# WangXinyan940/openmm-chargeflux

Measured on AMD Instinct MI355X. Metric: ns/day + ms/force-eval, periodic charge-flux box, 1/2/4/8 MI355X, higher is better.
Workload: dtype f64; 1 GPU; C3: periodic flexible charge-flux water box, 96000 atoms, Ewald rc=1.0 nm tol=0.0001 (alpha 2.91842, kmax 31, K_half 113490), velocity Verlet dt=1 fs, fp64; atoms=96000, k_half=113490, handover=event, variants=0, kspace=grid (ES kernel W=13, pruned DFT), same k-set, parallelism=atom-decomposition x1

## Files before the change

### openmm-chargeflux_amd/csrc/cf_api.hip

```cpp
#include <hip/hip_runtime.h>

#include <algorithm>
#include <cmath>
#include <cstring>
#include <exception>
#include <numeric>
#include <stdexcept>
#include <string>
#include <vector>

#include "cf_internal.h"

enum Phase { PH_FLUX, PH_PREP, PH_CELLS, PH_NLIST, PH_TABLES, PH_SFAC, PH_COEFFS, PH_FORCE, PH_DIRECT,
             PH_ASSEMBLE, PH_ENERGY, PH_GSORT, PH_GSPREAD, PH_GDFTF, PH_GDFTI, PH_GINTERP, PH_EXCL, PH_COUNT };
static const char* kPhaseNames[PH_COUNT] = {"flux_terms", "atoms_prep", "cell_sort", "neighbor_list",
                                            "kspace_tables", "kspace_sfac", "kspace_coeffs", "kspace_force",
                                            "direct_pairs", "assemble", "energy", "grid_sort", "grid_spread",
                                            "grid_dft_fwd", "grid_dft_inv", "grid_interp", "direct_excl"};
constexpr int kMaxTimed = 8192;

static void graph_forget(cf_handle* H);
static void graph_invalidate(cf_handle* H);
struct GraphCache;
static GraphCache* graph_active(cf_handle* H);
// ... 147 lines not shown

void set_cells(cf_handle* H, const double L[3]) {
    cf::Handle& h = H->h;
    const double bx = h.box_t[0], cx = h.box_t[1], cy = h.box_t[2];
    const double V = L[0] * L[1] * L[2];
    const double width[3] = {V / std::sqrt((L[1] * L[2]) * (L[1] * L[2]) + (bx * L[2]) * (bx * L[2]) +
                                           (bx * cy - L[1] * cx) * (bx * cy - L[1] * cx)),
                             L[1] * L[2] / std::sqrt(L[2] * L[2] + cy * cy), L[2]};
    int nc[3];
    for (int d = 0; d < 3; d++) {
        double v = std::floor((h.tric ? width[d] : L[d]) / (h.cutoff + h.list_skin));
        nc[d] = (int)std::max(1.0, std::min(v, 1024.0));
    }
    int64_t ncell = (int64_t)nc[0] * nc[1] * nc[2];
    if (ncell > h.ncell_alloc) {
        bump_epoch(H);
        if (h.cell_start) { free_idle(h, h.cell_start); free_idle(h, h.cell_end); free_idle(h, h.cell_cnt); }
        if (h.own_cnt) { free_idle(h, h.own_cnt); free_idle(h, h.own_start); h.own_cnt = h.own_start = nullptr; }
        zalloc((void**)&h.cell_start, sizeof(int) * ncell, "cells");
        zalloc((void**)&h.cell_end, sizeof(int) * ncell, "cells");
        zalloc((void**)&h.cell_cnt, sizeof(int) * ncell, "cells");
        if (h.world > 1) {
            zalloc((void**)&h.own_cnt, sizeof(int) * ncell, "cells");
            zalloc((void**)&h.own_start, sizeof(int) * (ncell + 1), "cells");
        }
        h.ncell_alloc = (int)ncell;
    }
    h.nc[0] = nc[0]; h.nc[1] = nc[1]; h.nc[2] = nc[2];
    if (h.nl) alloc_nlist(H, h.list_skin, L[0] * L[1] * L[2]);
    const double per_cell = (double)h.n / (double)ncell;
    const bool want_cluster = h.pair_list == CF_PAIR_LIST_CLUSTER || h.pair_list == CF_PAIR_LIST_AUTO;
    h.half = h.pair_list != CF_PAIR_LIST_FULL && h.pbc &&
             (h.world == 1 || (want_cluster && h.pair_list == CF_PAIR_LIST_CLUSTER)) && nc[0] >= 4 &&
             nc[1] >= 4 && nc[2] >= 4 && per_cell * 18.0 * 1.15 <= 4096.0 && h.n < (1 << 21);
    if (h.half && ncell > h.win_cells) {
        if (h.win_out) { free_idle(h, h.win_out); free_idle(h, h.win_woff); }
        zalloc((void**)&h.win_out, sizeof(unsigned long long) * 4 * 4096 * (size_t)ncell, "half-list windows");
        zalloc((void**)&h.win_woff, sizeof(int) * 18 * (size_t)ncell, "half-list windows");
        h.win_cells = (int)ncell;
        bump_epoch(H);
    }
    h.cluster = h.half && want_cluster;
    h.zcol = 0;
    if (h.cluster) {
        h.zcol = (int)std::max(1.0, std::min(8.0, std::round(std::sqrt(per_cell / 12.0))));
        const int need = h.n / 4 + (int)ncell + 1;
        const double rho = h.n / V;
        const double ext = 0.6 * std::cbrt(4.0 / rho);
        const double rl = h.cutoff + h.list_skin + ext;
        const double est = 0.5 * 4.0 / 3.0 * M_PI * rl * rl * rl * rho / 4.0 + 8.0;
        int cap = std::min(1536, ((int)(2.2 * est) + 64 + 15) / 16 * 16);
        if (h.list_capacity > 0) cap = std::max(4, std::min(cap, h.list_capacity));
        if (need > h.ncl_cap || cap != h.cpl_cap || ncell + 1 > h.cl_cells) {
            if (h.cl_start) { free_idle(h, h.cl_start); free_idle(h, h.cl_info); free_idle(h, h.cl_bb);
                              free_idle(h, h.cpl); free_idle(h, h.cpl_cnt); }
            h.ncl_cap = std::max(need, h.ncl_cap);
            h.cpl_cap = cap;
            h.cl_cells = std::max((int)ncell + 1, h.cl_cells);
            zalloc((void**)&h.cl_start, sizeof(int) * h.cl_cells, "cluster table");
            zalloc((void**)&h.cl_info, sizeof(int2) * h.ncl_cap, "cluster table");
            zalloc((void**)&h.cl_bb, sizeof(float4) * 2 * h.ncl_cap, "cluster table");
            zalloc((void**)&h.cpl, sizeof(uint2) * ((size_t)h.ncl_cap * h.cpl_cap + 64), "cluster-pair list");
            zalloc((void**)&h.cpl_cnt, sizeof(int) * h.ncl_cap, "cluster-pair list");
            bump_epoch(H);
        }
        if (!h.pos4f) {
            zalloc((void**)&h.pos4f, sizeof(float4) * (h.n + 4), "fp32 positions");
            zalloc((void**)&h.slot_of, sizeof(int) * h.n, "slot map");
            bump_epoch(H);
        }
    }
}

void set_box(cf_handle* H, const double* box9) {
    cf::Handle& h = H->h;
    if (!h.pbc) { h.box_L[0] = h.box_L[1] = h.box_L[2] = 1.0; return; }
    if (!box9) fail(CF_ERR_INVALID, "periodic box required");
    check_box_reduced(box9, "current box");
    double L[3] = {box9[0], box9[4], box9[8]};
    for (int d = 0; d < 3; d++)
        if (h.cutoff > 0.5 * L[d] * (1 + 1e-12))
            fail(CF_ERR_INVALID, "cutoff exceeds half the periodic box (minimum image would be ambiguous)");
    h.box_L[0] = L[0]; h.box_L[1] = L[1]; h.box_L[2] = L[2];
    h.box_t[0] = box9[3]; h.box_t[1] = box9[6]; h.box_t[2] = box9[7];
    h.tric = box9[3] != 0 || box9[6] != 0 || box9[7] != 0;
}

void partition(const cf_params* p, int world, int rank, int* lo, int* hi) {
    const int n = p->num_particles;
    if (world <= 1) { *lo = 0; *hi = n; return; }
    std::vector<int> par(n);
    std::iota(par.begin(), par.end(), 0);
    auto unite = [&](int a, int b) {
        if (a < 0 || a >= n || b < 0 || b >= n) fail(CF_ERR_INVALID, "particle index out of range");
        a = find_root(par, a); b = find_root(par, b);
        if (a != b) par[std::max(a, b)] = std::min(a, b);
    };
    for (int t = 0; t < p->num_flux_bonds; t++) unite(p->flux_bond_idx[2 * t], p->flux_bond_idx[2 * t + 1]);
    for (int t = 0; t < p->num_flux_angles; t++) {
        unite(p->flux_angle_idx[3 * t], p->flux_angle_idx[3 * t + 1]);
        unite(p->flux_angle_idx[3 * t], p->flux_angle_idx[3 * t + 2]);
    }
    for (int t = 0; t < p->num_flux_waters; t++) {
        unite(p->flux_water_idx[3 * t], p->flux_water_idx[3 * t + 1]);
        unite(p->flux_water_idx[3 * t], p->flux_water_idx[3 * t + 2]);
    }
    for (int k = 0; k < p->num_exceptions; k++) unite(p->exceptions[2 * k], p->exceptions[2 * k + 1]);
    std::vector<int> cmax(n, 0);
    for (int i = 0; i < n; i++) { int r = find_root(par, i); cmax[r] = std::max(cmax[r], i); }
    std::vector<char> valid(n + 1, 0);
    valid[0] = valid[n] = 1;
    int pm = -1;
    for (int c = 1; c < n; c++) {
        pm = std::max(pm, cmax[find_root(par, c - 1)]);
// ... 364 lines not shown
                h.g_t2 = dalloc<double2>(H, (size_t)gp.ng[0] * gp.NY * gp.KZ);
                h.g_b = dalloc<double2>(H, (size_t)gp.NX * gp.NY * gp.KZ);
                h.g_cnt = dalloc<int>(H, gp.nbins);
                check_hip(hipMemset(h.g_cnt, 0, sizeof(int) * gp.nbins), "memset");
                h.g_start = dalloc<int>(H, gp.nbins + 1);
                const size_t no = std::max(nown, 1);
                h.g_srec = dalloc<double4>(H, no);
                h.g_g0u = dalloc<int4>(H, no);
                h.g_rank = dalloc<int>(H, no);
                h.g_tmp = dalloc<int>(H, no);
                h.g_order = dalloc<int>(H, no);
                h.g_g0s = dalloc<int4>(H, no);
                h.g_taps = dalloc<double>(H, no * 72);
                check_hip(hipMemset(h.g_taps, 0, sizeof(double) * no * 72), "memset taps");
                if (h.world > 1) {
                    h.g_xrange = dalloc<int>(H, 3 + 2 * ((size_t)no / 256 + 1));
                    const int init[3] = {INT_MAX, INT_MIN, 0};
                    check_hip(hipMemcpy(h.g_xrange, init, sizeof(init), hipMemcpyHostToDevice), "x-slab init");
                }
                h.t_part = dalloc<double>(H, no * 4);
                h.e_rec_part = dalloc<double>(H, std::max<size_t>((size_t)(gp.NX * gp.NY * gp.KZ + 255) / 256,
                                                                  (size_t)gp.NY * gp.KZ / 16 + 2) + 1);
            } else {
                int blocks_k = (int)((h.khalf + 255) / 256);
                h.sk_nchunk = std::max(1, std::min((2048 + blocks_k - 1) / blocks_k, std::max(1, nown / 256)));
                h.kvec = dalloc<double4>(H, h.khalf);
                h.sk_slab = dalloc<double>(H, (size_t)h.sk_nchunk * 2 * h.khalf);
                h.sk_red = dalloc<double>(H, (size_t)2 * h.khalf);
                h.t_part = dalloc<double>(H, (size_t)nown * 4);
                h.e_rec_part = dalloc<double>(H, (size_t)(h.khalf + 255) / 256 + 1);
            }
        }
        check_hip(hipDeviceSynchronize(), "create sync");
        *out = H;
    });
    if (rc != CF_OK && H) {
        for (void* p2 : H->allocs) (void)hipFree(p2);
        if (H->h.err_host) (void)hipHostFree(H->h.err_host);
        delete H;
    }
    return rc;
}

CF_EXPORT int cf_destroy(cf_handle* H) {
    if (!H) return CF_OK;
    return guarded([&] {
        (void)hipSetDevice(H->h.device);
        drain_handle(H->h);
        graph_forget(H);
        for (void* p : H->allocs) (void)hipFree(p);
        for (auto& v : H->ev)
            for (hipEvent_t e : v) (void)hipEventDestroy(e);
        if (H->h.win_out) { (void)hipFree(H->h.win_out); (void)hipFree(H->h.win_woff); }
        if (H->h.cl_start) { (void)hipFree(H->h.cl_start); (void)hipFree(H->h.cl_info); (void)hipFree(H->h.cl_bb);
                             (void)hipFree(H->h.cpl); (void)hipFree(H->h.cpl_cnt); }
        if (H->h.pos4f) { (void)hipFree(H->h.pos4f); (void)hipFree(H->h.slot_of); }
        if (H->h.cell_start) (void)hipFree(H->h.cell_start);
        if (H->h.cell_end) (void)hipFree(H->h.cell_end);
        if (H->h.cell_cnt) (void)hipFree(H->h.cell_cnt);
        if (H->h.own_cnt) { (void)hipFree(H->h.own_cnt); (void)hipFree(H->h.own_start); }
        if (H->h.own_stream) (void)hipStreamDestroy(H->h.stream);
        if (H->h.aux) (void)hipStreamDestroy(H->h.aux);
        if (H->h.ev_fork) (void)hipEventDestroy(H->h.ev_fork);
        if (H->h.ev_join) (void)hipEventDestroy(H->h.ev_join);
        if (H->h.err_host) (void)hipHostFree(H->h.err_host);
        delete H;
    });
}

CF_EXPORT int cf_partition(const cf_params* p, int32_t world_size, int32_t rank, int32_t* lo, int32_t* hi) {
    return guarded([&] {
        if (!p || !lo || !hi) fail(CF_ERR_INVALID, "null argument");
        if (p->num_particles <= 0) fail(CF_ERR_INVALID, "num_particles must be > 0");
        int world = world_size <= 1 ? 1 : world_size;
        if (rank < 0 || rank >= world) fail(CF_ERR_INVALID, "rank out of range");
        int l = 0, h = 0;
        partition(p, world, rank, &l, &h);
        *lo = l; *hi = h;
    });
}

CF_EXPORT int cf_set_neighbor_skin(cf_handle* H, double skin) {
    return guarded([&] {
        if (!H) fail(CF_ERR_INVALID, "null handle");
        if (!(skin >= 0 && skin < 1e3)) fail(CF_ERR_INVALID, "skin must be finite and >= 0");
        cf::Handle& h = H->h;
        if (h.pending_flags >= 0) fail(CF_ERR_STATE, "cf_set_neighbor_skin during a begun evaluation");
        check_hip(hipSetDevice(h.device), "hipSetDevice");
        check_hip(hipStreamSynchronize(h.stream), "stream sync");
        h.skin = skin;
        h.list_valid = false;
        bump_epoch(H);
        if (!h.pbc) return;
        alloc_nlist(H, skin);
        if (skin > 0 && !h.pos_ref) h.pos_ref = dalloc<double>(H, (size_t)3 * h.n);
    });
}

CF_EXPORT int cf_update_parameters(cf_handle* H, const cf_params* p) {
    return guarded([&] {
        if (!H || !p) fail(CF_ERR_INVALID, "null argument");
        cf::Handle& h = H->h;
        if (h.pending_flags >= 0) fail(CF_ERR_STATE, "cf_update_parameters during a begun evaluation");
        if (p->num_particles != h.n) fail(CF_ERR_INVALID, "the number of particles has changed");
        if ((p->use_pbc ? 1 : 0) != h.pbc) fail(CF_ERR_INVALID, "periodicity cannot be changed by an update");
        if (h.pbc && (p->cutoff != h.cutoff || p->ewald_tol != h.tol))
            fail(CF_ERR_INVALID, "the cutoff and Ewald tolerance cannot be changed by an update");
// ... 865 lines not shown
```

### openmm-chargeflux_amd/csrc/cf_internal.h

```cpp
#pragma once

#include <hip/hip_runtime.h>
#include <stdint.h>

#include <string>
#include <vector>

#include "../../include/chargeflux.h"

namespace cf {

constexpr double kPi = 3.14159265358979323846;

struct KGeom {
    int KX = 0, KY = 0, KZ = 0;
    int NY = 0;
    int NYB = 0;
    int NYP = 0;
    int NYB4 = 0;
    int NMT = 0;
    int NZP = 0;
    int NB = 0;
    int CSW = 0;
    __host__ __device__ int nslots() const { return KX * NYP; }
// ... 88 lines not shown
    hipEvent_t ev_fork = nullptr, ev_join = nullptr;
    unsigned long long* sync_flag = nullptr;
    unsigned long long sync_seq = 0, join_seq = 0;
    bool handover_memory = false;
    double* dedq_rec = nullptr;
    double* f_rec = nullptr;
    int ncell_alloc = 0;
    int nc[3] = {0, 0, 0};
    int* cell_key = nullptr; int* cell_key_sorted = nullptr;
    int* atom_val = nullptr; int* atom_sorted = nullptr;
    int* cell_start = nullptr; int* cell_end = nullptr; int* cell_cnt = nullptr;
    double4* pos4s = nullptr;
    double2* ljs = nullptr;
    int lj_ntypes = 0;
    int* atom_type = nullptr;
    int* typ_s = nullptr;
    double2* lj_tab = nullptr;
    double skin = 0.0;
    double list_skin = 0.0;
    double list_L[3] = {0, 0, 0};
    double list_T[3] = {0, 0, 0};
    bool list_valid = false;
    double* pos_ref = nullptr;
    int* skin_flag = nullptr;
    long long* n_builds_dev = nullptr;
    long long* n_fallback_dev = nullptr;
    int64_t n_evals = 0;
    int* err_dev = nullptr;
    int* err_host = nullptr;
    int* err_host_dev = nullptr;
    int* key_tmp = nullptr; int* atom_tmp = nullptr;
    int* own_s = nullptr;
    int* own_cnt = nullptr;
    int* own_start = nullptr;
    int nb_cap = 0;
    int* nl = nullptr;
    int* nl_cnt = nullptr;
    bool half = false;
    int64_t alloc_epoch = 0;
    int* half_flag = nullptr;
    unsigned long long* win_out = nullptr;
    int* win_woff = nullptr;
    int win_cells = 0;
    bool cluster = false;
    int pair_list = CF_PAIR_LIST_AUTO;
    int list_capacity = 0;
    int variants = 0;
    int block_rounds() const { return (variants >> 8) & 15; }
    int zcol = 0;
    int ncl_cap = 0;
    int cl_cells = 0;
    int* cl_start = nullptr;
    int2* cl_info = nullptr;
    float4* cl_bb = nullptr;
    int cpl_cap = 0;
    uint2* cpl = nullptr;
    int* cpl_cnt = nullptr;
    float4* pos4f = nullptr;
    int* slot_of = nullptr;
    int npad = 0;
    double2* tab_xq = nullptr;
    double2* tab_y = nullptr;
    double* tab_cs = nullptr;
    double* s_slab = nullptr;
    double* s_red = nullptr;
    double* coef_a = nullptr;
    double* t_part = nullptr;
    double* e_rec_part = nullptr;
    int e_rec_nblk = 0;
    int coef_inv = 0;
    GridPlan gp;
    double* g_grid = nullptr;
    double2* g_t1 = nullptr;
    double2* g_t2 = nullptr;
    double2* g_b = nullptr;
    double2* g_tw[3] = {nullptr, nullptr, nullptr};
    double2* g_tw8[3] = {nullptr, nullptr, nullptr};
    double* g_deconv[3] = {nullptr, nullptr, nullptr};
    int* g_cnt = nullptr;
    int* g_start = nullptr;
    double4* g_srec = nullptr;
    int4* g_g0u = nullptr;
    int* g_rank = nullptr;
    int* g_tmp = nullptr;
    int* g_order = nullptr;
    int4* g_g0s = nullptr;
    double* g_taps = nullptr;
    int* g_xrange = nullptr;
    int64_t khalf = 0;
    double* sk_slab = nullptr;
    double* sk_red = nullptr;
    double4* kvec = nullptr;
    int sk_nchunk = 0;
    double* erfc_tab = nullptr;
    double erfc_scale = 0; int erfc_m = 0;
    double erfc_scale_f = 0; int erfc_m_f = 0;
    float* erfc_tab_f = nullptr;
    double* terms_dev = nullptr;
    double* e_part = nullptr;
    double* energy_dev = nullptr;
    int* e_ticket = nullptr;
    int pending_flags = -1;
    bool direct_done = false;
    double box_L[3] = {0, 0, 0};
    double box_t[3] = {0, 0, 0};
    bool tric = false;
};

std::vector<double> erfc_table(double xmax, double* scale, int* m);
std::vector<float> erfc_table_f(double xmax, double* scale, int* m);
std::vector<double> erfc_table_deg(double xmax, int deg, double width, int max_m, double* scale, int* m);
void launch_flux_terms(Handle& h, const double* pos);
void launch_atoms_prep(Handle& h, const double* pos, bool skin_check);
void launch_cell_sort(Handle& h, const double* pos);
void launch_force_rebuild(Handle& h);
void launch_zero(Handle& h, double* p, int64_t n);
void launch_nlist(Handle& h, const double* pos);
void launch_cluster_list(Handle& h);
void launch_pairs_cluster(Handle& h, const double* pos, int include_forces);
void launch_cluster_table(Handle& h);
void launch_direct(Handle& h, const double* pos, int include_forces);
void launch_direct_finish(Handle& h, const double* pos, int include_forces);
void launch_recip_add(Handle& h);
void launch_nopbc(Handle& h, const double* pos, int include_forces, int include_energy);
void launch_signal(Handle& h, unsigned long long* flag);
void launch_assemble_energy(Handle& h, double* forces_out, int include_energy, double* energy_out);

void kspace_plan(Handle& h);
size_t kspace_alloc_bytes(const Handle& h);
void launch_kspace_tables(Handle& h, const double* pos);
void launch_kspace_sfac(Handle& h);
double* kspace_reduce_buffer(Handle& h, int64_t* count);
void launch_kspace_coeffs(Handle& h, int include_energy);
void launch_kspace_force(Handle& h, const double* pos);

void launch_kspace_kvec(Handle& h);
void launch_kspace_direct_sfac(Handle& h, const double* pos);
void launch_kspace_direct_coeffs(Handle& h, int include_energy);
void launch_kspace_direct_force(Handle& h, const double* pos);

void grid_plan(Handle& h, int width, double sigma);
void grid_tables(const Handle& h, std::vector<double2> tw[3], std::vector<double2> tw8[3], std::vector<double> deconv[3]);
void launch_grid_sort(Handle& h, const double* pos);
void launch_grid_spread(Handle& h);
void launch_grid_dft_fwd(Handle& h);
double* grid_reduce_buffer(Handle& h, int64_t* count);
void launch_grid_coeffs(Handle& h, int include_energy, bool inverse_follows);
void launch_grid_dft_inv(Handle& h);
void launch_grid_interp(Handle& h, bool split = false);

void launch_om_gather(Handle& h, const void* posq, const void* corr, int posq_kind, const int* atom_index,
                      double* pos);
void launch_om_scatter(Handle& h, const int* atom_index, const double* frc, int padded, long long* fbuf,
                       const double* ene, void* ebuf, int energy_kind);

void check_hip(hipError_t e, const char* what);

#if defined(__HIP_DEVICE_COMPILE__)
#define CF_LDS_UNPAIRED __attribute__((target("no-load-store-opt")))
#else
#define CF_LDS_UNPAIRED
#endif

__device__ __forceinline__ double rsqrt_fp64(double r2) {
    double y = __builtin_amdgcn_rsq(r2);
    return y * fma(-0.5 * r2 * y, y, 1.5);
}

__device__ __forceinline__ double fma3(double a, double b, double c) {
    double d;
    asm("v_fma_f64 %0, %1, %2, %3" : "=v"(d) : "v"(a), "v"(b), "s"(c));
    return d;
}
// ... 148 lines not shown
```

### openmm-chargeflux_amd/csrc/cf_kernels_cluster.hip

```cpp
#include <type_traits>

#include "cf_pair.h"

namespace cf {

constexpr int kClSize = 4;
constexpr int kCqWaves = 16;
constexpr int kCqThreads = 64 * kCqWaves;
constexpr int kCqQ = kCqWaves > 12 ? 88 : 112;
constexpr int kCqBatch = 16;
constexpr int kCqLpi = 16;
constexpr int kClBuildThreads = 512;
constexpr int kClMaxCand = 1536;
constexpr unsigned kClSelfMask = 0x08CEu;
typedef float v2f __attribute__((ext_vector_type(2)));

__device__ __forceinline__ int window_cell(int k, int cx, int cy, int cz, int3 nc, double3 L, double3 T,
                                           float4& off, double3* wrap = nullptr) {
    const int3 o = half_offset(k);
    const int u[3] = {cx + o.x, cy + o.y, cz + o.z}, n[3] = {nc.x, nc.y, nc.z};
    int w[3], m[3];
#pragma unroll
    for (int d = 0; d < 3; d++) {
        m[d] = u[d] >= n[d] ? 1 : (u[d] < 0 ? -1 : 0);
        w[d] = u[d] - m[d] * n[d];
    }
    const double3 v = lattice(L, T, (double)o.x / nc.x, (double)o.y / nc.y, (double)o.z / nc.z);
    off = make_float4((float)v.x, (float)v.y, (float)v.z, 0.f);
    if (wrap) *wrap = lattice(L, T, m[0], m[1], m[2]);
    return (w[0] * nc.y + w[1]) * nc.z + w[2];
}

__global__ void __launch_bounds__(1024) k_cl_scan(int ncell, const int* __restrict__ flag, const int* __restrict__ cstart,
                                                  const int* __restrict__ cend, int* __restrict__ cl_start, int ncl_cap,
                                                  int* __restrict__ err) {
    __shared__ int sh[1024];
    if (!*flag) return;
    int carry = 0;
    for (int base = 0; base < ncell; base += 1024) {
        const int c = base + threadIdx.x;
        const int v = c < ncell ? (cend[c] - cstart[c] + kClSize - 1) / kClSize : 0;
        const int x = block_exclusive_scan_t<1024>(v, sh);
        if (c < ncell) cl_start[c] = carry + x;
        carry += sh[1023];
        __syncthreads();
    }
    if (threadIdx.x == 0) {
        cl_start[ncell] = carry;
        if (carry > ncl_cap) atomicOr(err, kGuardClusterTable);
    }
}

__global__ void __launch_bounds__(256) k_cl_bbox(int ncell, const int* __restrict__ flag, const int* __restrict__ cstart,
                                                 const int* __restrict__ cend, const int* __restrict__ cl_start,
                                                 const float4* __restrict__ pos4f, int2* __restrict__ cl_info,
                                                 float4* __restrict__ cl_bb, int3 nc, double3 L, double3 T,
                                                 const int* __restrict__ atom_sorted, int lo, int hi, int n,
                                                 int ncl_cap) {
    const int lane = threadIdx.x & 63;
    const int c = blockIdx.x * 4 + (threadIdx.x >> 6);
    if (c >= ncell || !*flag) return;
    const int b = cstart[c], e = cend[c], k0 = cl_start[c];
    if (cl_start[c + 1] > ncl_cap) return;
    const double ox = lattice(L, T, (double)(c / (nc.y * nc.z)) / nc.x, (double)((c / nc.z) % nc.y) / nc.y,
                              (double)(c % nc.z) / nc.z).x;
    for (int k = lane; k * kClSize < e - b; k += 64) {
        const int first = b + k * kClSize, cnt = min(kClSize, e - first);
        float4 bl = pos4f[first], bh = bl;
        bool own = lo == 0 && hi == n;
        for (int u = 0; u < cnt; u++) {
            const float4 p = pos4f[first + u];
            bl.x = fminf(bl.x, p.x); bl.y = fminf(bl.y, p.y); bl.z = fminf(bl.z, p.z);
            bh.x = fmaxf(bh.x, p.x); bh.y = fmaxf(bh.y, p.y); bh.z = fmaxf(bh.z, p.z);
            const int ai = atom_sorted[first + u];
            own = own || (ai >= lo && ai < hi);
        }
        cl_info[k0 + k] = make_int2(first, cnt);
        bl.w = (float)(ox + 0.5 * ((double)bl.x + (double)bh.x));
        bh.w = own ? 1.f : 0.f;
        cl_bb[2 * (k0 + k)] = bl;
        cl_bb[2 * (k0 + k) + 1] = bh;
    }
}

__global__ void __launch_bounds__(kClBuildThreads) k_cl_build(DirectArgs a, const float4* __restrict__ cl_bb,
                                                              uint2* __restrict__ cpl, int* __restrict__ cpl_cnt,
                                                              float rlm2) {
    __shared__ float4 cand_lo[kClMaxCand], cand_hi[kClMaxCand];
    __shared__ float cand_x[kClMaxCand];
    __shared__ int woff[kHalfWin + 1];
    __shared__ int wcl[kHalfWin];
    __shared__ float4 wsh[kHalfWin];
    __shared__ int exs[kClBuildThreads / 64][64];
    if (!*a.flag) return;
    const int cell = xcd_block();
    const int3 nc = a.nc;
    const int cz = cell % nc.z, cy = (cell / nc.z) % nc.y, cx = cell / (nc.y * nc.z);
    if (threadIdx.x < kHalfWin) {
        float4 off;
        wcl[threadIdx.x] = window_cell(threadIdx.x, cx, cy, cz, nc, a.L, a.T, off);
        wsh[threadIdx.x] = off;
    }
    __syncthreads();
    if (threadIdx.x == 0) {
        int off = 0;
        for (int k = 0; k < kHalfWin; k++) {
            woff[k] = off;
            off += a.cl_start[wcl[k] + 1] - a.cl_start[wcl[k]];
        }
        woff[kHalfWin] = off;
    }
    __syncthreads();
    const int ncand = woff[kHalfWin];
    if (ncand > kClMaxCand) {
        if (threadIdx.x == 0) atomicOr(a.half_flag, kHalfWindowFull);
        for (int ci = a.cl_start[cell] + threadIdx.x; ci < a.cl_start[cell + 1]; ci += kClBuildThreads)
            cpl_cnt[ci] = a.cpl_cap + 1;
        return;
    }
    for (int t = threadIdx.x; t < ncand; t += kClBuildThreads) {
        int k = 0;
        while (woff[k + 1] <= t) k++;
        const int cj = a.cl_start[wcl[k]] + (t - woff[k]);
        const float4 sh = wsh[k];
        const float4 lo = cl_bb[2 * cj], hi = cl_bb[2 * cj + 1];
        const int first = a.cl_info[cj].x;
        const unsigned ownj = hi.w != 0.f ? 0x80000000u : 0u;
        cand_lo[t] = make_float4(lo.x + sh.x, lo.y + sh.y, lo.z + sh.z,
                                 __int_as_float((int)((unsigned)cj | ((unsigned)(a.cl_info[cj].y - 1) << 29) | ownj)));
        cand_hi[t] = make_float4(hi.x + sh.x, hi.y + sh.y, hi.z + sh.z, __int_as_float(first | (k << kHalfSlotBits)));
        cand_x[t] = lo.w;
    }
    __syncthreads();
    const int lane = threadIdx.x & 63, wv = threadIdx.x >> 6;
    const int c0 = a.cl_start[cell], c1 = a.cl_start[cell + 1];
    if (c1 > a.ncl_cap) return;
    for (int ci = c0 + wv; ci < c1; ci += kClBuildThreads / 64) {
        const float4 ilo = cl_bb[2 * ci], ihi = cl_bb[2 * ci + 1];
        const float xki = ilo.w;
        const bool owni = ihi.w != 0.f;
        const int2 ii = a.cl_info[ci];
        const unsigned rows = (1u << (4 * ii.y)) - 1u;
        uint2* out = cpl + (size_t)ci * a.cpl_cap;
        int cnt = 0;
        int nex = 0;
        bool many = false;
        int exlo = INT_MAX, exhi = INT_MIN;
        {
            const int il = lane >> 4, e = lane & 15;
            int v = -1;
            if (il < ii.y) {
                const int ai = a.atom_sorted[ii.x + il];
                const int e0 = a.ex_start[ai], ne = a.ex_start[ai + 1] - e0;
                many = ne > 16;
                if (e < ne) v = (il << 24) | a.slot_of[a.ex_list[e0 + e]];
            }
            many = __ballot(many) != 0;
            const unsigned long long has = __ballot(v >= 0);
            const int r = __popcll(has & ((1ull << lane) - 1ull));
            if (v >= 0) exs[wv][r] = v;
            nex = __popcll(has);
            int mn = v >= 0 ? (v & 0xFFFFFF) : INT_MAX, mx = v >= 0 ? (v & 0xFFFFFF) : INT_MIN;
#pragma unroll
            for (int o = 32; o > 0; o >>= 1) {
                mn = min(mn, __shfl_xor(mn, o));
                mx = max(mx, __shfl_xor(mx, o));
            }
            exlo = __builtin_amdgcn_readfirstlane(mn);
            exhi = __builtin_amdgcn_readfirstlane(mx);
            __builtin_amdgcn_fence(__ATOMIC_RELEASE, "wavefront");
            __builtin_amdgcn_wave_barrier();
            __builtin_amdgcn_fence(__ATOMIC_ACQUIRE, "wavefront");
        }
        for (int t0 = 0; t0 < ncand; t0 += 64) {
            const int t = t0 + lane;
            bool hit = false;
            unsigned mask = 0;
            int ent = 0;
            if (t < ncand) {
                const float4 lo = cand_lo[t], hi = cand_hi[t];
                const float dx = fmaxf(0.f, fmaxf(lo.x - ihi.x, ilo.x - hi.x));
                const float dy = fmaxf(0.f, fmaxf(lo.y - ihi.y, ilo.y - hi.y));
                const float dz = fmaxf(0.f, fmaxf(lo.z - ihi.z, ilo.z - hi.z));
                const int cj = __float_as_int(lo.w) & 0x1FFFFFFF;
                ent = __float_as_int(hi.w);
                const int k = ent >> kHalfSlotBits;
                const float xkj = cand_x[t];
                const bool ownj = (unsigned)__float_as_int(lo.w) >> 31;
                if (dx * dx + dy * dy + dz * dz <= rlm2 && (k >= 9 || xkj > xki || (xkj == xki && cj >= ci)) &&
                    (owni || ownj)) {
                    const int jcnt = (((unsigned)__float_as_int(lo.w) >> 29) & 3u) + 1;
                    const unsigned cols = 0x1111u * ((1u << jcnt) - 1u);
                    mask = rows & cols & (cj == ci ? kClSelfMask : 0xFFFFu);
                    hit = true;
// ... 291 lines not shown
                    qbuf[wv][k][ring((int)x)] = word;
                }
            }
            q0 += cnt[0]; q1 += cnt[1]; q2 += cnt[2]; q3 += cnt[3];
            if (!pf_ok && all_ge(kCqLpi)) issue_pf();
            while (all_ge(2 * kCqLpi)) phase_b();
            en_c = en_n; pj_c = pj_n; en_n = en_nn;
        }
        while (q0 > 0 || q1 > 0 || q2 > 0 || q3 > 0) phase_b();
#pragma unroll
        for (int m = 1; m < kCqLpi; m <<= 1) {
            acc.fx += __shfl_xor(acc.fx, m); acc.fy += __shfl_xor(acc.fy, m); acc.fz += __shfl_xor(acc.fz, m);
            acc.dq += __shfl_xor(acc.dq, m); acc.e += __shfl_xor(acc.e, m);
        }
        const int i = a.atom_sorted[islot];
        if (kk == 0 && il < inf.y && i >= a.lo && i < a.hi) {
            a.e_atom[3 * i + 1] = acc.e;
            if (a.include_forces) {
                a.dedq[i] = acc.dq;
                if constexpr (MIXED) {
                    a.f_part[3 * i] = acc.fx * -(double)kFix32Inv;
                    a.f_part[3 * i + 1] = acc.fy * -(double)kFix32Inv;
                    a.f_part[3 * i + 2] = acc.fz * -(double)kFix32Inv;
                } else {
                    a.f_part[3 * i] = acc.fx * -kFixInv;
                    a.f_part[3 * i + 1] = acc.fy * -kFixInv;
                    a.f_part[3 * i + 2] = acc.fz * -kFixInv;
                }
            }
        }
    }
    if (!a.include_forces) return;
    __syncthreads();
    if constexpr (MIXED) {
        uint4* out = reinterpret_cast<uint4*>(a.win_out) + (size_t)cell * kHalfMaxWin;
        for (int e = threadIdx.x; e < nw; e += kCqThreads) out[e] = make_uint4(accw[0][e], accw[1][e], accw[2][e], accw[3][e]);
    } else {
        unsigned long long* out = a.win_out + (size_t)cell * kHalfMaxWin * 4;
        for (int e = threadIdx.x; e < nw; e += kCqThreads)
            reinterpret_cast<ulonglong4*>(out)[e] = make_ulonglong4(accw[0][e], accw[1][e], accw[2][e], accw[3][e]);
    }
    };
    process(cell0 + xcd_block());
    {
        const int why = (__ballot(bad_list) ? kHalfListOverflow : 0) | (__ballot(bad) ? kHalfFixedRange : 0);
        if (why && lane == 0) atomicOr(a.half_flag, why);
        if (__ballot(bad_idx) && lane == 0) {
            atomicOr(a.half_flag, kHalfListOverflow);
            atomicOr(a.err, kGuardListEntry);
        }
    }
}

void launch_cluster_table(Handle& h) {
    DirectArgs a = direct_args(h, nullptr, 0);
    const int ncell = h.nc[0] * h.nc[1] * h.nc[2];
    hipLaunchKernelGGL(k_cl_scan, dim3(1), dim3(1024), 0, h.stream, ncell, h.skin_flag, h.cell_start, h.cell_end,
                       h.cl_start, h.ncl_cap, h.err_dev);
    hipLaunchKernelGGL(k_cl_bbox, dim3((ncell + 3) / 4), dim3(256), 0, h.stream, ncell, h.skin_flag, h.cell_start,
                       h.cell_end, h.cl_start, h.pos4f, h.cl_info, h.cl_bb, make_int3(h.nc[0], h.nc[1], h.nc[2]),
                       make_double3(h.box_L[0], h.box_L[1], h.box_L[2]), make_double3(h.box_t[0], h.box_t[1], h.box_t[2]),
                       a.atom_sorted, a.lo, a.hi, a.n, h.ncl_cap);
}

void launch_cluster_list(Handle& h) {
    DirectArgs a = direct_args(h, nullptr, 0);
    const int ncell = h.nc[0] * h.nc[1] * h.nc[2];
    launch_cluster_table(h);
    const double rl = (h.cutoff + h.list_skin) * (1.0 + 1e-5) + 1e-5;
    hipLaunchKernelGGL(k_cl_build, dim3(ncell), dim3(kClBuildThreads), 0, h.stream, a, h.cl_bb, h.cpl, h.cpl_cnt,
                       (float)(rl * rl));
}

void launch_pairs_cluster(Handle& h, const double* pos, int include_forces) {
    DirectArgs a = direct_args(h, pos, include_forces);
    const int ncell = h.nc[0] * h.nc[1] * h.nc[2];
#define CF_PAIRS_CQ(TY_, MX_) hipLaunchKernelGGL((k_pairs_cq<TY_, MX_>), dim3(ncell), dim3(kCqThreads), 0, h.stream, a, 0)
    if (h.mixed) {
        if (a.typ_s) CF_PAIRS_CQ(true, true);
        else CF_PAIRS_CQ(false, true);
    } else {
        if (a.typ_s) CF_PAIRS_CQ(true, false);
        else CF_PAIRS_CQ(false, false);
    }
#undef CF_PAIRS_CQ
}

}
```

### openmm-chargeflux_amd/csrc/cf_kernels_core.hip

```cpp
#include <algorithm>
#include <type_traits>

#include "cf_pair.h"

namespace cf {


__device__ __forceinline__ long dqdx_start(int t, int nb, int na) {
    const int b = min(t, nb), an = max(0, min(t, nb + na) - nb), w = max(0, t - nb - na);
    return 3L * (4L * b + 9L * an + 9L * w);
}

__global__ void __launch_bounds__(256) k_flux_terms(int nterms, int nb, int na, const int4* __restrict__ tidx,
                                                    const double* __restrict__ tpar, const double* __restrict__ pos,
                                                    double3 L, double3 T, int pbc, double* __restrict__ dq_slot,
                                                    double* __restrict__ dqdx) {
    __shared__ double st[256 * 27];
    const int t0 = blockIdx.x * blockDim.x;
    const int t = t0 + threadIdx.x;
    const long base = dqdx_start(t0, nb, na);
    if (t < nterms) {
        int4 ti = tidx[t];
        const double* p = tpar + 5 * t;
        double* o = st + (dqdx_start(t, nb, na) - base);
// ... 54 lines not shown
                o[0 + j] = a12k1 + a12k2 + a13k1 + a13k2;
                o[3 + j] = -a12k1 - a12k2 + 2 * ub;
                o[6 + j] = -a13k2 - a13k1 - 2 * ub;
                o[9 + j] = -a12k1 - a13k2;
                o[12 + j] = a12k1 - ub;
                o[15 + j] = a13k2 + ub;
                o[18 + j] = -a12k2 - a13k1;
                o[21 + j] = a12k2 - ub;
                o[24 + j] = a13k1 + ub;
            }
        }
    }
    __syncthreads();
    const int len = (int)(dqdx_start(min(t0 + (int)blockDim.x, nterms), nb, na) - base);
    for (int e = threadIdx.x; e < len; e += blockDim.x) dqdx[base + e] = st[e];
}
__global__ void __launch_bounds__(256) k_atoms_prep(int n, const double* __restrict__ q0,
                                                    const int* __restrict__ qs, const int* __restrict__ qslot,
                                                    const double* __restrict__ dq_slot, int pbc, double alpha, double ke,
                                                    double* __restrict__ q, double* __restrict__ dedq_self,
                                                    double* __restrict__ e_atom, const double* __restrict__ pos,
                                                    const double* __restrict__ pos_ref, double lim2,
                                                    int* __restrict__ skin_flag) {
    int i = blockIdx.x * blockDim.x + threadIdx.x;
    if (skin_flag) {
        bool moved = false;
        if (i < n) {
            double3 x = ld3(pos, i), r = ld3(pos_ref, i);
            double dx = x.x - r.x, dy = x.y - r.y, dz = x.z - r.z;
            moved = !(dx * dx + dy * dy + dz * dz <= lim2);
        }
        if (__ballot(moved) && (threadIdx.x & 63) == 0) atomicOr(skin_flag, 1);
    }
    if (i >= n) return;
    double qi = q0[i];
    for (int s = qs[i]; s < qs[i + 1]; s++) qi += dq_slot[qslot[s]];
    q[i] = qi;
    if (pbc) {
        const double c = ke * alpha / sqrt(kPi);
        dedq_self[i] = -2 * c * qi;
        e_atom[3 * i] = -c * qi * qi;
    } else {
        dedq_self[i] = 0;
        e_atom[3 * i] = 0;
    }
}


__global__ void __launch_bounds__(256) k_cell_hist(int n, const int* __restrict__ flag, const double* __restrict__ pos,
                                                   double3 L, double3 T, int3 nc, int* __restrict__ key, int* __restrict__ rank,
                                                   int* __restrict__ cnt, int* __restrict__ ticket,
                                                   int* __restrict__ cstart, int* __restrict__ cend, int lo, int hi,
                                                   int* __restrict__ own_cnt, int* __restrict__ own_start,
                                                   int* __restrict__ err) {
    __shared__ int sh[256];
    if (!*flag) return;
    const int i = blockIdx.x * blockDim.x + threadIdx.x;
    const bool valid = i < n;
    int k = 0;
    if (valid) {
        const double3 x = ld3(pos, i);
        const double3 wp = wrap_by(x, floor3(fractional(x, L, T)), L, T);
        const double3 f = fractional(wp, L, T);
        const double fs[3] = {f.x, f.y, f.z};
        int ncs[3] = {nc.x, nc.y, nc.z};
        int c[3];
#pragma unroll
        for (int d = 0; d < 3; d++) {
            int ci = (int)(fs[d] * ncs[d]);
            c[d] = ci < 0 ? 0 : (ci >= ncs[d] ? ncs[d] - 1 : ci);
        }
        k = (c[0] * nc.y + c[1]) * nc.z + c[2];
        key[i] = k;
    }
    const int r = wave_agg_inc(cnt, k, valid);
    if (valid) rank[i] = r;
    if (own_cnt) (void)wave_agg_inc(own_cnt, k, valid && i >= lo && i < hi);
    if (!last_block_done(ticket)) return;
    const int ncell = nc.x * nc.y * nc.z;
    const int total = block_counts_to_bounds<256>(ncell, cnt, cstart, cend, false, sh);
    if (total != n) {
        __syncthreads();
        for (int c = threadIdx.x; c < ncell; c += blockDim.x) { cstart[c] = 0; cend[c] = 0; }
        if (threadIdx.x == 0) atomicOr(err, kGuardCellBounds);
    }
    if (own_cnt) {
        __syncthreads();
        block_counts_to_bounds<256>(nc.x * nc.y * nc.z, own_cnt, own_start, nullptr, true, sh);
    }
}

__global__ void __launch_bounds__(256) k_cell_scatter(int n, const int* __restrict__ flag, const int* __restrict__ key,
                                                      const int* __restrict__ rank, const int* __restrict__ cstart,
                                                      int* __restrict__ tmp, int ncell, int* __restrict__ cnt,
                                                      int* __restrict__ own_cnt, int* __restrict__ err) {
    int i = blockIdx.x * blockDim.x + threadIdx.x;
    if (!*flag) return;
    for (int c = i; c < ncell; c += gridDim.x * blockDim.x) {
        cnt[c] = 0;
        if (own_cnt) own_cnt[c] = 0;
    }
    if (i >= n) return;
    const int k = key[i], s = (unsigned)k < (unsigned)ncell ? cstart[k] + rank[i] : -1;
    if ((unsigned)s >= (unsigned)n) { atomicOr(err, kGuardCellBounds); return; }
    tmp[s] = i;
}

constexpr int kOrderLds = 1024;

__global__ void __launch_bounds__(256) k_cell_order(int ncell, const int* __restrict__ flag,
                                                    const int* __restrict__ cstart, const int* __restrict__ cend,
                                                    const int* __restrict__ tmp, int* __restrict__ out, int lo, int hi,
                                                    const int* __restrict__ own_start, int* __restrict__ own_s,
                                                    const double* __restrict__ pos, double3 L, double3 T, int3 nc,
                                                    int zcol, int n, int* __restrict__ err) {
    __shared__ unsigned long long memk[kOrderLds];
    const int tid = threadIdx.x;
    const int c = blockIdx.x;
    if (c >= ncell || !*flag) return;
    const int b = cstart[c], m = cend[c] - b;
    if (b < 0 || m < 0 || b + m > n) {
        if (tid == 0) atomicOr(err, kGuardCellBounds);
        return;
    }
    const int* src = tmp + b;
    if (m > kOrderLds) {
        for (int e = tid; e < m; e += 256) {
            const int v = src[e];
            int r = 0, ro = 0;
            for (int j = 0; j < m; j++) {
                const int u = src[j];
                r += u < v;
                if (own_s) ro += u < v && u >= lo && u < hi;
            }
            out[b + r] = v;
            if (own_s && v >= lo && v < hi) own_s[own_start[c] + ro] = b + r;
        }
// ... 1217 lines not shown
    for (int i = 0; i < M; i++) {
        std::vector<long double> f(n), c(n, 0.0L);
        for (int k = 0; k < n; k++) {
            const long double t = cosl(3.14159265358979323846264338327950288L * (k + 0.5L) / n);
            const long double x = w * (i + 0.5L * (t + 1.0L));
            f[k] = erfcl(x) * expl(x * x);
        }
        for (int j = 0; j < n; j++) {
            long double sum = 0;
            for (int k = 0; k < n; k++)
                sum += f[k] * cosl(3.14159265358979323846264338327950288L * j * (k + 0.5L) / n);
            c[j] = (j == 0 ? 1.0L : 2.0L) * sum / n;
        }
        std::vector<std::vector<long double>> T(n, std::vector<long double>(n, 0.0L));
        T[0][0] = 1.0L;
        if (n > 1) T[1][1] = 1.0L;
        for (int j = 1; j + 1 < n; j++)
            for (int e = 0; e < n; e++) T[j + 1][e] = (e > 0 ? 2.0L * T[j][e - 1] : 0.0L) - T[j - 1][e];
        for (int e = 0; e < n; e++) {
            long double v = 0;
            for (int j = 0; j < n; j++) v += c[j] * T[j][e];
            tab[(size_t)i * n + e] = (double)v;
        }
    }
    *scale = (double)(1.0L / w);
    *m = M;
    return tab;
}

void launch_flux_terms(Handle& h, const double* pos) {
    if (h.nterms == 0) return;
    double3 L = make_double3(h.box_L[0], h.box_L[1], h.box_L[2]);
    hipLaunchKernelGGL(k_flux_terms, dim3(nblk(h.nterms, 256)), dim3(256), 0, h.stream, h.nterms, h.nb, h.na,
                       h.term_idx, h.term_par, pos, L, make_double3(h.box_t[0], h.box_t[1], h.box_t[2]), h.pbc,
                       h.dq_slot, h.dqdx);
}

void launch_atoms_prep(Handle& h, const double* pos, bool skin_check) {
    const double lim = 0.5 * h.list_skin;
    hipLaunchKernelGGL(k_atoms_prep, dim3(nblk(h.n, 256)), dim3(256), 0, h.stream, h.n, h.q0, h.qcsr_start,
                       h.qcsr_slot, h.dq_slot, h.pbc, h.alpha, h.ke, h.q, h.dedq_self, h.e_atom, pos, h.pos_ref, lim * lim,
                       skin_check ? h.skin_flag : nullptr);
}

void launch_cell_sort(Handle& h, const double* pos) {
    double3 L = make_double3(h.box_L[0], h.box_L[1], h.box_L[2]);
    int3 nc = make_int3(h.nc[0], h.nc[1], h.nc[2]);
    int ncell = nc.x * nc.y * nc.z;
    const int* f = h.skin_flag;
    int* oc = h.own_s ? h.own_cnt : nullptr;
    const double3 T = make_double3(h.box_t[0], h.box_t[1], h.box_t[2]);
    hipLaunchKernelGGL(k_cell_hist, dim3(nblk(h.n, 256)), dim3(256), 0, h.stream, h.n, f, pos, L, T, nc, h.cell_key,
                       h.atom_val, h.cell_cnt, h.e_ticket + kTicketCells, h.cell_start, h.cell_end, h.lo, h.hi, oc,
                       h.own_start, h.err_dev);
    hipLaunchKernelGGL(k_cell_scatter, dim3(nblk(h.n, 256)), dim3(256), 0, h.stream, h.n, f, h.cell_key, h.atom_val,
                       h.cell_start, h.atom_tmp, ncell, h.cell_cnt, oc, h.err_dev);
    hipLaunchKernelGGL(k_cell_order, dim3(ncell), dim3(256), 0, h.stream, ncell, f, h.cell_start,
                       h.cell_end, h.atom_tmp, h.key_tmp, h.lo, h.hi, h.own_start, oc ? h.own_s : nullptr, pos, L, T,
                       nc, h.zcol, h.n, h.err_dev);
    hipLaunchKernelGGL(k_cell_commit, dim3(nblk(h.n, 256)), dim3(256), 0, h.stream, h.n, f, h.cell_key, h.key_tmp,
                       pos, h.q, h.lj, L, T, h.cell_key_sorted, h.atom_sorted, h.pos4s, h.ljs,
                       h.atom_type, h.typ_s,
                       h.pos_ref, h.n_builds_dev, h.cluster ? h.pos4f : nullptr, h.cluster ? h.slot_of : nullptr, nc,
                       h.err_dev);
}

__global__ void k_set_flag(int* __restrict__ flag) {
    if (threadIdx.x == 0) *flag = 1;
}

void launch_force_rebuild(Handle& h) {
    hipLaunchKernelGGL(k_set_flag, dim3(1), dim3(64), 0, h.stream, h.skin_flag);
}

__global__ void __launch_bounds__(256) k_zero(double* __restrict__ p, int64_t n) {
    for (int64_t i = (int64_t)blockIdx.x * blockDim.x + threadIdx.x; i < n; i += (int64_t)gridDim.x * blockDim.x) p[i] = 0.0;
}

void launch_zero(Handle& h, double* p, int64_t n) {
    if (n <= 0) return;
    hipLaunchKernelGGL(k_zero, dim3((unsigned)std::min<int64_t>((n + 255) / 256, 2048)), dim3(256), 0, h.stream, p, n);
}

DirectArgs direct_args(Handle& h, const double* pos, int include_forces) {
    DirectArgs a;
    a.n = h.n; a.lo = h.lo; a.hi = h.hi; a.include_forces = include_forces;
    a.L = make_double3(h.box_L[0], h.box_L[1], h.box_L[2]);
    a.T = make_double3(h.box_t[0], h.box_t[1], h.box_t[2]);
    a.tric = h.tric ? 1 : 0;
    a.invL = make_double3(1.0 / h.box_L[0], 1.0 / h.box_L[1], 1.0 / h.box_L[2]);
    a.nc = make_int3(h.nc[0], h.nc[1], h.nc[2]);
    a.brute = (h.nc[0] < 3 || h.nc[1] < 3 || h.nc[2] < 3) ? 1 : 0;
    a.rc2 = h.cutoff * h.cutoff; a.rc = h.cutoff; a.alpha = h.alpha; a.ke = h.ke;
    a.erfc_tab = h.erfc_tab; a.erfc_scale = h.erfc_scale; a.erfc_m = h.erfc_m;
    a.erfc_tab_f = h.erfc_tab_f; a.erfc_scale_f = h.erfc_scale_f; a.erfc_m_f = h.erfc_m_f;
    a.rl2 = (h.cutoff + h.list_skin) * (h.cutoff + h.list_skin);
    a.nb_cap = h.nb_cap;
    a.nlr = h.hi - h.lo;
    a.own_s = h.own_s;
    a.own_start = h.world > 1 ? h.own_start : nullptr;
    a.flag = h.skin_flag;
    a.atom_sorted = h.atom_sorted; a.key_sorted = h.cell_key_sorted;
    a.cstart = h.cell_start; a.cend = h.cell_end;
    a.pos4s = h.pos4s; a.ljs = h.ljs;
    a.typ_s = h.typ_s; a.lj_tab = h.lj_tab; a.lj_ntypes = h.lj_ntypes;
    a.q = h.q; a.ex_start = h.ex_start; a.ex_list = h.ex_list;
    a.dedq_self = h.dedq_self;
// ... 115 lines not shown
```

Baseline: 199.7 ns/day.

## Fold cluster table scan into cell histogram and compute bounding boxes in list build

Removes the separate cluster-start scan kernel and the cluster bounding-box kernel. The cluster prefix scan now runs inside the last block of the cell histogram kernel, and the list-build kernel computes candidate cluster boxes on the fly from cell bounds and fp32 positions. It also derives cluster info for its own cell from the shared candidate arrays instead of reading a cl_bb buffer. This saves two launches and a global round trip on each rebuild, at the cost of recomputing boxes redundantly across neighbouring cells' build blocks and a longer serial tail in the histogram kernel.

```diff
diff --git a/openmm-chargeflux_amd/csrc/cf_api.hip b/openmm-chargeflux_amd/csrc/cf_api.hip
--- a/openmm-chargeflux_amd/csrc/cf_api.hip
+++ b/openmm-chargeflux_amd/csrc/cf_api.hip
@@ -223,14 +223,13 @@
         int cap = std::min(1536, ((int)(2.2 * est) + 64 + 15) / 16 * 16);
         if (h.list_capacity > 0) cap = std::max(4, std::min(cap, h.list_capacity));
         if (need > h.ncl_cap || cap != h.cpl_cap || ncell + 1 > h.cl_cells) {
-            if (h.cl_start) { free_idle(h, h.cl_start); free_idle(h, h.cl_info); free_idle(h, h.cl_bb);
+            if (h.cl_start) { free_idle(h, h.cl_start); free_idle(h, h.cl_info);
                               free_idle(h, h.cpl); free_idle(h, h.cpl_cnt); }
             h.ncl_cap = std::max(need, h.ncl_cap);
             h.cpl_cap = cap;
             h.cl_cells = std::max((int)ncell + 1, h.cl_cells);
             zalloc((void**)&h.cl_start, sizeof(int) * h.cl_cells, "cluster table");
             zalloc((void**)&h.cl_info, sizeof(int2) * h.ncl_cap, "cluster table");
-            zalloc((void**)&h.cl_bb, sizeof(float4) * 2 * h.ncl_cap, "cluster table");
             zalloc((void**)&h.cpl, sizeof(uint2) * ((size_t)h.ncl_cap * h.cpl_cap + 64), "cluster-pair list");
             zalloc((void**)&h.cpl_cnt, sizeof(int) * h.ncl_cap, "cluster-pair list");
             bump_epoch(H);
@@ -701,7 +700,7 @@
         for (auto& v : H->ev)
             for (hipEvent_t e : v) (void)hipEventDestroy(e);
         if (H->h.win_out) { (void)hipFree(H->h.win_out); (void)hipFree(H->h.win_woff); }
-        if (H->h.cl_start) { (void)hipFree(H->h.cl_start); (void)hipFree(H->h.cl_info); (void)hipFree(H->h.cl_bb);
+        if (H->h.cl_start) { (void)hipFree(H->h.cl_start); (void)hipFree(H->h.cl_info);
                              (void)hipFree(H->h.cpl); (void)hipFree(H->h.cpl_cnt); }
         if (H->h.pos4f) { (void)hipFree(H->h.pos4f); (void)hipFree(H->h.slot_of); }
         if (H->h.cell_start) (void)hipFree(H->h.cell_start);
diff --git a/openmm-chargeflux_amd/csrc/cf_internal.h b/openmm-chargeflux_amd/csrc/cf_internal.h
--- a/openmm-chargeflux_amd/csrc/cf_internal.h
+++ b/openmm-chargeflux_amd/csrc/cf_internal.h
@@ -164,7 +164,6 @@
     int cl_cells = 0;
     int* cl_start = nullptr;
     int2* cl_info = nullptr;
-    float4* cl_bb = nullptr;
     int cpl_cap = 0;
     uint2* cpl = nullptr;
     int* cpl_cnt = nullptr;
@@ -230,7 +229,6 @@
 void launch_nlist(Handle& h, const double* pos);
 void launch_cluster_list(Handle& h);
 void launch_pairs_cluster(Handle& h, const double* pos, int include_forces);
-void launch_cluster_table(Handle& h);
 void launch_direct(Handle& h, const double* pos, int include_forces);
 void launch_direct_finish(Handle& h, const double* pos, int include_forces);
 void launch_recip_add(Handle& h);
diff --git a/openmm-chargeflux_amd/csrc/cf_kernels_cluster.hip b/openmm-chargeflux_amd/csrc/cf_kernels_cluster.hip
--- a/openmm-chargeflux_amd/csrc/cf_kernels_cluster.hip
+++ b/openmm-chargeflux_amd/csrc/cf_kernels_cluster.hip
@@ -13,6 +13,7 @@
 constexpr int kClBuildThreads = 512;
 constexpr int kClMaxCand = 1536;
 constexpr unsigned kClSelfMask = 0x08CEu;
+constexpr int kOwnWin = 4;
 typedef float v2f __attribute__((ext_vector_type(2)));
 
 __device__ __forceinline__ int window_cell(int k, int cx, int cy, int cz, int3 nc, double3 L, double3 T,
@@ -31,65 +32,44 @@
     return (w[0] * nc.y + w[1]) * nc.z + w[2];
 }
 
-__global__ void __launch_bounds__(1024) k_cl_scan(int ncell, const int* __restrict__ flag, const int* __restrict__ cstart,
-                                                  const int* __restrict__ cend, int* __restrict__ cl_start, int ncl_cap,
-                                                  int* __restrict__ err) {
-    __shared__ int sh[1024];
-    if (!*flag) return;
-    int carry = 0;
-    for (int base = 0; base < ncell; base += 1024) {
-        const int c = base + threadIdx.x;
-        const int v = c < ncell ? (cend[c] - cstart[c] + kClSize - 1) / kClSize : 0;
-        const int x = block_exclusive_scan_t<1024>(v, sh);
-        if (c < ncell) cl_start[c] = carry + x;
-        carry += sh[1023];
-        __syncthreads();
-    }
-    if (threadIdx.x == 0) {
-        cl_start[ncell] = carry;
-        if (carry > ncl_cap) atomicOr(err, kGuardClusterTable);
-    }
-}
-
-__global__ void __launch_bounds__(256) k_cl_bbox(int ncell, const int* __restrict__ flag, const int* __restrict__ cstart,
-                                                 const int* __restrict__ cend, const int* __restrict__ cl_start,
-                                                 const float4* __restrict__ pos4f, int2* __restrict__ cl_info,
-                                                 float4* __restrict__ cl_bb, int3 nc, double3 L, double3 T,
-                                                 const int* __restrict__ atom_sorted, int lo, int hi, int n,
-                                                 int ncl_cap) {
-    const int lane = threadIdx.x & 63;
-    const int c = blockIdx.x * 4 + (threadIdx.x >> 6);
-    if (c >= ncell || !*flag) return;
-    const int b = cstart[c], e = cend[c], k0 = cl_start[c];
-    if (cl_start[c + 1] > ncl_cap) return;
-    const double ox = lattice(L, T, (double)(c / (nc.y * nc.z)) / nc.x, (double)((c / nc.z) % nc.y) / nc.y,
-                              (double)(c % nc.z) / nc.z).x;
-    for (int k = lane; k * kClSize < e - b; k += 64) {
-        const int first = b + k * kClSize, cnt = min(kClSize, e - first);
-        float4 bl = pos4f[first], bh = bl;
-        bool own = lo == 0 && hi == n;
+__device__ __forceinline__ int2 cluster_box(const DirectArgs& a, int b, int e, int k, double ox, float4& bl,
+                                            float4& bh) {
+    const int first = b + k * kClSize, cnt = min(kClSize, e - first);
+    float4 p[kClSize];
+#pragma unroll
+    for (int u = 0; u < kClSize; u++) p[u] = a.pos4f[first + u];
+    bl = p[0];
+    bh = bl;
+#pragma unroll
+    for (int u = 1; u < kClSize; u++)
+        if (u < cnt) {
+            bl.x = fminf(bl.x, p[u].x); bl.y = fminf(bl.y, p[u].y); bl.z = fminf(bl.z, p[u].z);
+            bh.x = fmaxf(bh.x, p[u].x); bh.y = fmaxf(bh.y, p[u].y); bh.z = fmaxf(bh.z, p[u].z);
+        }
+    bool own = a.lo == 0 && a.hi == a.n;
+    if (!own)
         for (int u = 0; u < cnt; u++) {
-            const float4 p = pos4f[first + u];
-            bl.x = fminf(bl.x, p.x); bl.y = fminf(bl.y, p.y); bl.z = fminf(bl.z, p.z);
-            bh.x = fmaxf(bh.x, p.x); bh.y = fmaxf(bh.y, p.y); bh.z = fmaxf(bh.z, p.z);
-            const int ai = atom_sorted[first + u];
-            own = own || (ai >= lo && ai < hi);
-        }
-        cl_info[k0 + k] = make_int2(first, cnt);
-        bl.w = (float)(ox + 0.5 * ((double)bl.x + (double)bh.x));
-        bh.w = own ? 1.f : 0.f;
-        cl_bb[2 * (k0 + k)] = bl;
-        cl_bb[2 * (k0 + k) + 1] = bh;
-    }
-}
-
-__global__ void __launch_bounds__(kClBuildThreads) k_cl_build(DirectArgs a, const float4* __restrict__ cl_bb,
+            const int ai = a.atom_sorted[first + u];
+            own = own || (ai >= a.lo && ai < a.hi);
+        }
+    bl.w = (float)(ox + 0.5 * ((double)bl.x + (double)bh.x));
+    bh.w = own ? 1.f : 0.f;
+    return make_int2(first, cnt);
+}
+__device__ __forceinline__ double cell_corner_x(int c, int3 nc, double3 L, double3 T) {
+    return lattice(L, T, (double)(c / (nc.y * nc.z)) / nc.x, (double)((c / nc.z) % nc.y) / nc.y,
+                   (double)(c % nc.z) / nc.z).x;
+}
+
+__global__ void __launch_bounds__(kClBuildThreads) k_cl_build(DirectArgs a, int2* __restrict__ cl_info,
                                                               uint2* __restrict__ cpl, int* __restrict__ cpl_cnt,
                                                               float rlm2) {
     __shared__ float4 cand_lo[kClMaxCand], cand_hi[kClMaxCand];
     __shared__ float cand_x[kClMaxCand];
     __shared__ int woff[kHalfWin + 1];
     __shared__ int wcl[kHalfWin];
+    __shared__ int2 wbe[kHalfWin];
+    __shared__ double wox[kHalfWin];
     __shared__ float4 wsh[kHalfWin];
     __shared__ int exs[kClBuildThreads / 64][64];
     if (!*a.flag) return;
@@ -98,7 +78,10 @@
     const int cz = cell % nc.z, cy = (cell / nc.z) % nc.y, cx = cell / (nc.y * nc.z);
     if (threadIdx.x < kHalfWin) {
         float4 off;
-        wcl[threadIdx.x] = window_cell(threadIdx.x, cx, cy, cz, nc, a.L, a.T, off);
+        const int w = window_cell(threadIdx.x, cx, cy, cz, nc, a.L, a.T, off);
+        wcl[threadIdx.x] = w;
+        wbe[threadIdx.x] = make_int2(a.cstart[w], a.cend[w]);
+        wox[threadIdx.x] = cell_corner_x(w, nc, a.L, a.T);
         wsh[threadIdx.x] = off;
     }
     __syncthreads();
@@ -106,16 +89,23 @@
         int off = 0;
         for (int k = 0; k < kHalfWin; k++) {
             woff[k] = off;
-            off += a.cl_start[wcl[k] + 1] - a.cl_start[wcl[k]];
+            off += (wbe[k].y - wbe[k].x + kClSize - 1) / kClSize;
         }
         woff[kHalfWin] = off;
     }
     __syncthreads();
+    const int lane = threadIdx.x & 63, wv = threadIdx.x >> 6;
+    const int cb = a.cstart[cell], ce = a.cend[cell];
+    const int c0 = a.cl_start[cell], c1 = c0 + (ce - cb + kClSize - 1) / kClSize;
+    if (c1 > a.ncl_cap) return;
     const int ncand = woff[kHalfWin];
     if (ncand > kClMaxCand) {
         if (threadIdx.x == 0) atomicOr(a.half_flag, kHalfWindowFull);
-        for (int ci = a.cl_start[cell] + threadIdx.x; ci < a.cl_start[cell + 1]; ci += kClBuildThreads)
+        for (int ci = c0 + threadIdx.x; ci < c1; ci += kClBuildThreads) {
+            const int first = cb + (ci - c0) * kClSize;
+            cl_info[ci] = make_int2(first, min(kClSize, ce - first));
             cpl_cnt[ci] = a.cpl_cap + 1;
+        }
         return;
     }
     for (int t = threadIdx.x; t < ncand; t += kClBuildThreads) {
@@ -123,23 +113,23 @@
         while (woff[k + 1] <= t) k++;
         const int cj = a.cl_start[wcl[k]] + (t - woff[k]);
         const float4 sh = wsh[k];
-        const float4 lo = cl_bb[2 * cj], hi = cl_bb[2 * cj + 1];
-        const int first = a.cl_info[cj].x;
+        float4 lo, hi;
+        const int2 ij = cluster_box(a, wbe[k].x, wbe[k].y, t - woff[k], wox[k], lo, hi);
         const unsigned ownj = hi.w != 0.f ? 0x80000000u : 0u;
         cand_lo[t] = make_float4(lo.x + sh.x, lo.y + sh.y, lo.z + sh.z,
-                                 __int_as_float((int)((unsigned)cj | ((unsigned)(a.cl_info[cj].y - 1) << 29) | ownj)));
-        cand_hi[t] = make_float4(hi.x + sh.x, hi.y + sh.y, hi.z + sh.z, __int_as_float(first | (k << kHalfSlotBits)));
+                                 __int_as_float((int)((unsigned)cj | ((unsigned)(ij.y - 1) << 29) | ownj)));
+        cand_hi[t] = make_float4(hi.x + sh.x, hi.y + sh.y, hi.z + sh.z, __int_as_float(ij.x | (k << kHalfSlotBits)));
         cand_x[t] = lo.w;
     }
     __syncthreads();
-    const int lane = threadIdx.x & 63, wv = threadIdx.x >> 6;
-    const int c0 = a.cl_start[cell], c1 = a.cl_start[cell + 1];
-    if (c1 > a.ncl_cap) return;
     for (int ci = c0 + wv; ci < c1; ci += kClBuildThreads / 64) {
-        const float4 ilo = cl_bb[2 * ci], ihi = cl_bb[2 * ci + 1];
-        const float xki = ilo.w;
-        const bool owni = ihi.w != 0.f;
-        const int2 ii = a.cl_info[ci];
+        const int ti = woff[kOwnWin] + (ci - c0);
+        const float4 ilo = cand_lo[ti], ihi = cand_hi[ti];
+        const float xki = cand_x[ti];
+        const unsigned iw = (unsigned)__float_as_int(ilo.w);
+        const bool owni = iw >> 31;
+        const int2 ii = make_int2(__float_as_int(ihi.w) & kHalfSlotMask, (int)((iw >> 29) & 3u) + 1);
+        if (lane == 0) cl_info[ci] = ii;
         const unsigned rows = (1u << (4 * ii.y)) - 1u;
         uint2* out = cpl + (size_t)ci * a.cpl_cap;
         int cnt = 0;
@@ -537,23 +527,11 @@
     }
 }
 
-void launch_cluster_table(Handle& h) {
-    DirectArgs a = direct_args(h, nullptr, 0);
-    const int ncell = h.nc[0] * h.nc[1] * h.nc[2];
-    hipLaunchKernelGGL(k_cl_scan, dim3(1), dim3(1024), 0, h.stream, ncell, h.skin_flag, h.cell_start, h.cell_end,
-                       h.cl_start, h.ncl_cap, h.err_dev);
-    hipLaunchKernelGGL(k_cl_bbox, dim3((ncell + 3) / 4), dim3(256), 0, h.stream, ncell, h.skin_flag, h.cell_start,
-                       h.cell_end, h.cl_start, h.pos4f, h.cl_info, h.cl_bb, make_int3(h.nc[0], h.nc[1], h.nc[2]),
-                       make_double3(h.box_L[0], h.box_L[1], h.box_L[2]), make_double3(h.box_t[0], h.box_t[1], h.box_t[2]),
-                       a.atom_sorted, a.lo, a.hi, a.n, h.ncl_cap);
-}
-
 void launch_cluster_list(Handle& h) {
     DirectArgs a = direct_args(h, nullptr, 0);
     const int ncell = h.nc[0] * h.nc[1] * h.nc[2];
-    launch_cluster_table(h);
     const double rl = (h.cutoff + h.list_skin) * (1.0 + 1e-5) + 1e-5;
-    hipLaunchKernelGGL(k_cl_build, dim3(ncell), dim3(kClBuildThreads), 0, h.stream, a, h.cl_bb, h.cpl, h.cpl_cnt,
+    hipLaunchKernelGGL(k_cl_build, dim3(ncell), dim3(kClBuildThreads), 0, h.stream, a, h.cl_info, h.cpl, h.cpl_cnt,
                        (float)(rl * rl));
 }
 
diff --git a/openmm-chargeflux_amd/csrc/cf_kernels_core.hip b/openmm-chargeflux_amd/csrc/cf_kernels_core.hip
--- a/openmm-chargeflux_amd/csrc/cf_kernels_core.hip
+++ b/openmm-chargeflux_amd/csrc/cf_kernels_core.hip
@@ -130,7 +130,7 @@
                                                    int* __restrict__ cnt, int* __restrict__ ticket,
                                                    int* __restrict__ cstart, int* __restrict__ cend, int lo, int hi,
                                                    int* __restrict__ own_cnt, int* __restrict__ own_start,
-                                                   int* __restrict__ err) {
+                                                   int* __restrict__ err, int* __restrict__ cl_start, int ncl_cap) {
     __shared__ int sh[256];
     if (!*flag) return;
     const int i = blockIdx.x * blockDim.x + threadIdx.x;
@@ -161,6 +161,30 @@
         __syncthreads();
         for (int c = threadIdx.x; c < ncell; c += blockDim.x) { cstart[c] = 0; cend[c] = 0; }
         if (threadIdx.x == 0) atomicOr(err, kGuardCellBounds);
+    }
+    if (cl_start) {
+        int carry = 0;
+        for (int base = 0; base < ncell; base += 4 * 256) {
+            int v[4], sum = 0;
+#pragma unroll
+            for (int u = 0; u < 4; u++) {
+                const int c = base + 4 * threadIdx.x + u;
+                v[u] = (c < ncell && total == n) ? (ld_agent(cnt + c) + 3) / 4 : 0;
+                sum += v[u];
+            }
+            int run = carry + block_exclusive_scan_t<256>(sum, sh);
+            carry += sh[255];
+#pragma unroll
+            for (int u = 0; u < 4; u++) {
+                const int c = base + 4 * threadIdx.x + u;
+                if (c < ncell) cl_start[c] = run;
+                run += v[u];
+            }
+        }
+        if (threadIdx.x == 0) {
+            cl_start[ncell] = carry;
+            if (carry > ncl_cap) atomicOr(err, kGuardClusterTable);
+        }
     }
     if (own_cnt) {
         __syncthreads();
@@ -1484,7 +1508,7 @@
     const double3 T = make_double3(h.box_t[0], h.box_t[1], h.box_t[2]);
     hipLaunchKernelGGL(k_cell_hist, dim3(nblk(h.n, 256)), dim3(256), 0, h.stream, h.n, f, pos, L, T, nc, h.cell_key,
                        h.atom_val, h.cell_cnt, h.e_ticket + kTicketCells, h.cell_start, h.cell_end, h.lo, h.hi, oc,
-                       h.own_start, h.err_dev);
+                       h.own_start, h.err_dev, h.cluster ? h.cl_start : nullptr, h.ncl_cap);
     hipLaunchKernelGGL(k_cell_scatter, dim3(nblk(h.n, 256)), dim3(256), 0, h.stream, h.n, f, h.cell_key, h.atom_val,
                        h.cell_start, h.atom_tmp, ncell, h.cell_cnt, oc, h.err_dev);
     hipLaunchKernelGGL(k_cell_order, dim3(ncell), dim3(256), 0, h.stream, ncell, f, h.cell_start,
```

New measurement: 199.3 ns/day (median of 2 runs). No clear change (-0.2%).
